# EvolEcolGroup/tidypopgen

Hardware: AMD Instinct MI355X
Metric: SNP-genotypes/s (N x M) for IBS+KING+GRM+Fst+PCA; max |delta| vs CPU ref (cpu_baseline.parity) (higher is better)
Workload: dtype fp4-e2m1 operands (exact integers, f32 accumulate) for the cross-products, the PCA Gram and the grouped counts, int8 (int32 accumulate) for the loadings, f64 for statistics

## Files before the change

### tidypopgen_amd/csrc/fst.hip

```cpp
#include <math.h>

#include <algorithm>

#include "common.h"
#include "devfrag.h"
#include "fst_terms.h"
#include "host/host_fsttiles.h"
typedef double v2d __attribute__((ext_vector_type(2)));

template <int METHOD, bool FAST, int PPT>
__global__ __launch_bounds__(256) void tpg_fst_kernel(FstSrc src, int64_t m, int G, int LB,
                                                      const int32_t* __restrict__ pairs0, int P, int by_locus,
                                                      int return_num_dem, double* __restrict__ part,
                                                      double* __restrict__ out_a, double* __restrict__ out_b) {
  extern __shared__ __attribute__((aligned(16))) double sh[];
  double* sh_n = sh;
  double* sh_p = sh + (size_t)LB * G;
  double* sh_h = sh + 2 * (size_t)LB * G;
  double* sh_e = sh + 3 * (size_t)LB * G;
  int pidx[PPT], g1[PPT], g2[PPT];
  double sum_num[PPT], sum_den[PPT];
#pragma unroll
  for (int k = 0; k < PPT; k++) {
    pidx[k] = (blockIdx.y * PPT + k) * 256 + threadIdx.x;
    g1[k] = 0; g2[k] = 0;
    if (pidx[k] < P) { g1[k] = pairs0[2 * pidx[k]]; g2[k] = pairs0[2 * pidx[k] + 1]; }
    sum_num[k] = 0.0; sum_den[k] = 0.0;
  }
  const int64_t nchunks = (m + LB - 1) / LB;
  for (int64_t ch = blockIdx.x; ch < nchunks; ch += gridDim.x) {
    const int64_t j0 = ch * LB;
    __syncthreads();
    for (int idx = threadIdx.x; idx < LB * G; idx += 256) {
      const int l = idx / G, g = idx % G;
      const int64_t j = j0 + l;
      double vn = FST_NAN, vp = FST_NAN, vh = FST_NAN;
      if (j < m) fst_stage(src, m, j, g, vn, vp, vh);
      sh_n[idx] = vn; sh_p[idx] = vp; sh_h[idx] = vh;
      if (METHOD == TPG_FST_HUDSON) sh_e[idx] = (vp * (1 - vp)) / (vn - 1);
      if (METHOD == TPG_FST_WC84 && FAST) {
        const double ni = 0.5 * vn;
        sh_n[idx] = ni; sh_h[idx] = vh * ni; sh_e[idx] = 1.0 / ni;
      }
    }
    __syncthreads();
    const int lmax = (int)((m - j0) < LB ? (m - j0) : LB);
#pragma unroll
    for (int k = 0; k < PPT; k++) {
      if (pidx[k] >= P) continue;
#pragma unroll 2
      for (int l = 0; l < lmax; l++) {
        const int o1 = l * G + g1[k], o2 = l * G + g2[k];
        double num, den;
        constexpr bool use_e = METHOD == TPG_FST_HUDSON || (METHOD == TPG_FST_WC84 && FAST);
        fst_terms<METHOD, FAST>(sh_n[o1], sh_p[o1], sh_h[o1], use_e ? sh_e[o1] : 0.0, sh_n[o2], sh_p[o2], sh_h[o2],
                                use_e ? sh_e[o2] : 0.0, num, den);
        if (!FAST && by_locus) {
          const int64_t o = (j0 + l) + (int64_t)pidx[k] * m;
          if (!return_num_dem) out_a[o] = num / den;
          else { out_a[o] = num; out_b[o] = den; }
        }
        if (num == num && den == den) { sum_num[k] += num; sum_den[k] += den; }
      }
    }
  }
#pragma unroll
  for (int k = 0; k < PPT; k++)
    if (pidx[k] < P) {
      part[((int64_t)blockIdx.x * P + pidx[k]) * 2] = sum_num[k];
      part[((int64_t)blockIdx.x * P + pidx[k]) * 2 + 1] = sum_den[k];
    }
}

__global__ __launch_bounds__(256) void tpg_fst_reduce_kernel(const double* __restrict__ part, int nblocks, int P,
                                                             double* __restrict__ fst_tot, double* __restrict__ sum_num,
                                                             double* __restrict__ sum_den) {
  __shared__ double shn[16][17], shd[16][17];
  const int px = threadIdx.x & 15, sl = threadIdx.x >> 4;
  const int pi = blockIdx.x * 16 + px;
  double sn = 0.0, sd = 0.0;
  if (pi < P)
    for (int b = sl; b < nblocks; b += 16) { sn += part[((int64_t)b * P + pi) * 2]; sd += part[((int64_t)b * P + pi) * 2 + 1]; }
  shn[sl][px] = sn; shd[sl][px] = sd;
  __syncthreads();
  if (sl == 0 && pi < P) {
    sn = 0.0; sd = 0.0;
    for (int t = 0; t < 16; t++) { sn += shn[t][px]; sd += shd[t][px]; }
    if (fst_tot) fst_tot[pi] = sn / sd;
    if (sum_num) { sum_num[pi] = sn; sum_den[pi] = sd; }
  }
}

#define FSTG_T 64
#define FSTG_LB 16
#define FSTG_RS_MFMA 80
__global__ __launch_bounds__(256) void tpg_fst_hudson_gemm_kernel(FstSrc src, int64_t m, int G, int ntile, int kmax,
                                                                  double* __restrict__ part) {
  extern __shared__ __attribute__((aligned(16))) double sh[];
  constexpr int RS = FSTG_RS_MFMA;
  double* ra = sh;
  double* rc = sh + FSTG_LB * RS;
  double* cb = sh + 2 * FSTG_LB * RS;
  const int tR = blockIdx.y / ntile, tC = blockIdx.y % ntile;
  const bool diag = tR == tC;
  double* cc = diag ? rc : sh + 3 * FSTG_LB * RS;
  double* inv = sh + 4 * FSTG_LB * RS;
  for (int A = threadIdx.x; A <= kmax; A += 256) { inv[2 * A] = 1.0 / (double)A; inv[2 * A + 1] = 1.0 / ((double)A - 1.0); }
  double AB[4][4], CB[4][4], CC[4][4];
#pragma unroll
  for (int r = 0; r < 4; r++)
#pragma unroll
    for (int c = 0; c < 4; c++) { AB[r][c] = 0.0; CB[r][c] = 0.0; CC[r][c] = 0.0; }
  const int lane = threadIdx.x & 63, wv = threadIdx.x >> 6, r16 = lane & 15, kq = lane >> 4;
  const int64_t nchunks = (m + FSTG_LB - 1) / FSTG_LB;
  constexpr int NSLOT = 2 * FSTG_LB * FSTG_T / 256;
  const int nslot = (diag ? 1 : 2) * FSTG_LB * FSTG_T / 256;
  int pn1[NSLOT], pn2[NSLOT], pnv[NSLOT];
  auto fetch = [&](int64_t ch) {
#pragma unroll
    for (int i = 0; i < NSLOT; i++) {
      pn1[i] = 0; pn2[i] = 0; pnv[i] = 0;
      if (i < nslot && ch < nchunks) {
        const int idx = threadIdx.x + 256 * i;
        const int side = idx / (FSTG_LB * FSTG_T), rem = idx % (FSTG_LB * FSTG_T);
        const int g = (side ? tC : tR) * FSTG_T + rem % FSTG_T;
        const int64_t j = ch * FSTG_LB + rem / FSTG_T;
        if (j < m && g < G) {
          const int64_t plane = src.Mpad * src.Cpad, o = j * src.Cpad + g;
          pn1[i] = src.cnt[o]; pn2[i] = src.cnt[plane + o]; pnv[i] = src.cnt[2 * plane + o];
        }
      }
    }
  };
  if (kmax > 0) fetch(blockIdx.x);
  for (int64_t ch = blockIdx.x; ch < nchunks; ch += gridDim.x) {
    const int64_t j0 = ch * FSTG_LB;
    __syncthreads();
    if (kmax > 0) {
#pragma unroll
      for (int i = 0; i < NSLOT; i++) {
        if (i >= nslot) break;
        const int idx = threadIdx.x + 256 * i;
        const int side = idx / (FSTG_LB * FSTG_T), rem = idx % (FSTG_LB * FSTG_T);
        double a = 0.0, b = 0.0, c = 0.0;
        const int A = min(2 * pnv[i], kmax);
        if (A > 0) {
          const double vp = (double)(pn1[i] + 2 * pn2[i]) * inv[2 * A];
          const double e = (vp * (1 - vp)) * inv[2 * A + 1];
          if (e == e) { a = vp * vp - e; b = 1.0; c = vp; }
        }
        const int srem = (rem / FSTG_T) * RS + rem % FSTG_T;
        if (side) { cb[srem] = b; cc[srem] = c; }
        else {
          ra[srem] = a; rc[srem] = c;
          if (diag) cb[srem] = b;
        }
      }
    } else {
      for (int idx = threadIdx.x; idx < (diag ? 1 : 2) * FSTG_LB * FSTG_T; idx += 256) {
        const int side = idx / (FSTG_LB * FSTG_T), rem = idx % (FSTG_LB * FSTG_T);
        const int l = rem / FSTG_T, gl = rem % FSTG_T;
        const int g = (side ? tC : tR) * FSTG_T + gl;
        const int64_t j = j0 + l;
        double a = 0.0, b = 0.0, c = 0.0;
        if (j < m && g < G) {
          double vn, vp, vh;
          fst_stage(src, m, j, g, vn, vp, vh);
          const double e = (vp * (1 - vp)) / (vn - 1);
          if (vp == vp && e == e) { a = vp * vp - e; b = 1.0; c = vp; }
        }
        const int srem = l * RS + gl;
        if (side) { cb[srem] = b; cc[srem] = c; }
        else {
          ra[srem] = a; rc[srem] = c;
          if (diag) cb[srem] = b;
        }
      }
    }
    __syncthreads();
    if (kmax > 0) fetch(ch + gridDim.x);
#pragma unroll
    for (int l = 0; l < FSTG_LB; l += 4) {
      const double av = ra[(l + kq) * RS + 16 * wv + r16], cv = rc[(l + kq) * RS + 16 * wv + r16];
#pragma unroll
      for (int ct = 0; ct < 4; ct++) {
        const double bv = cb[(l + kq) * RS + 16 * ct + r16], dv = cc[(l + kq) * RS + 16 * ct + r16];
        *(v4d*)AB[ct] = __builtin_amdgcn_mfma_f64_16x16x4f64(av, bv, *(v4d*)AB[ct], 0, 0, 0);
        *(v4d*)CB[ct] = __builtin_amdgcn_mfma_f64_16x16x4f64(cv, bv, *(v4d*)CB[ct], 0, 0, 0);
        *(v4d*)CC[ct] = __builtin_amdgcn_mfma_f64_16x16x4f64(cv, dv, *(v4d*)CC[ct], 0, 0, 0);
      }
    }
  }
  double* o = part + (((int64_t)blockIdx.x * gridDim.y + blockIdx.y) * 3) * FSTG_T * FSTG_T;
#pragma unroll
  for (int ct = 0; ct < 4; ct++)
#pragma unroll
    for (int reg = 0; reg < 4; reg++) {
      const int q = (16 * wv + kq + 4 * reg) * FSTG_T + 16 * ct + r16;
      o[q] = AB[ct][reg];
      o[FSTG_T * FSTG_T + q] = CB[ct][reg];
      o[2 * FSTG_T * FSTG_T + q] = CC[ct][reg];
    }
}

#define FSTG_SL 16
__global__ __launch_bounds__(256) void tpg_fst_hudson_gemm_reduce_kernel(const double* __restrict__ part, int nbx, int64_t cells,
                                                                         double* __restrict__ full) {
  const int64_t q = blockIdx.x * (int64_t)blockDim.x + threadIdx.x;
  if (q >= cells) return;
  double s = 0.0;
  for (int b = blockIdx.y; b < nbx; b += FSTG_SL) s += part[(int64_t)b * cells + q];
  full[(int64_t)blockIdx.y * cells + q] = s;
}

__global__ void tpg_fst_hudson_gemm_final_kernel(const double* __restrict__ full, int64_t cells, int ntile,
                                                 const int32_t* __restrict__ pairs0, int P, double* __restrict__ fst_tot,
                                                 double* __restrict__ sum_num, double* __restrict__ sum_den) {
  const int pi = blockIdx.x * blockDim.x + threadIdx.x;
  if (pi >= P) return;
  const int g1 = pairs0[2 * pi], g2 = pairs0[2 * pi + 1];
  auto at = [&](int prod, int r, int c) {
    const int t = (r / FSTG_T) * ntile + c / FSTG_T;
    const int64_t q = (((int64_t)t * 3 + prod) * FSTG_T + r % FSTG_T) * FSTG_T + c % FSTG_T;
    double v = 0.0;
    for (int sl = 0; sl < FSTG_SL; sl++) v += full[(int64_t)sl * cells + q];
    return v;
  };
  const double cc2 = 2 * at(2, g1, g2);
  const double sn = at(0, g1, g2) + at(0, g2, g1) - cc2, sd = at(1, g1, g2) + at(1, g2, g1) - cc2;
  if (fst_tot) fst_tot[pi] = sn / sd;
  if (sum_num) { sum_num[pi] = sn; sum_den[pi] = sd; }
}

#define FSTW_TAB 4
template <int PPT, int GS>
__global__ __launch_bounds__(256) void tpg_fst_wc84_tab_kernel(FstSrc src, int64_t m, int G, int LB, int kmax,
                                                               const int32_t* __restrict__ pairs0, int P,
                                                               double* __restrict__ part) {
  extern __shared__ __attribute__((aligned(16))) double sh[];
  const int gs = GS ? GS : G;
  const uint32_t sb_b = (uint32_t)LB * gs * 16u, tab_b = (uint32_t)LB * gs * 32u, tab2_b = tab_b + (uint32_t)(kmax + 1) * 16u;
  char* shb = (char*)sh;
  for (int A = threadIdx.x; A <= kmax; A += 256) {
    const double nt = 0.5 * (double)A, nb1 = 0.5 * nt - 1.0;
    const double r = 1.0 / nt, sv = 1.0 / nb1;
    double* t = (double*)(shb + tab_b) + (size_t)A * 2;
    t[0] = r;
    t[1] = (0.5 * (nt - 1.0)) * r;
    double* t2 = (double*)(shb + tab2_b) + (size_t)A * 2;
    t2[0] = (0.5 * nt) * sv;
    t2[1] = (0.25 * (nt * nt)) * sv;
  }
  int pidx[PPT];
  uint32_t o1[PPT], o2[PPT];
  double sum_num[PPT], sum_den[PPT];
#pragma unroll
  for (int k = 0; k < PPT; k++) {
    pidx[k] = (blockIdx.y * PPT + k) * 256 + threadIdx.x;
    o1[k] = 0; o2[k] = 0;
    if (pidx[k] < P) { o1[k] = (uint32_t)pairs0[2 * pidx[k]]; o2[k] = (uint32_t)pairs0[2 * pidx[k] + 1]; }
    sum_num[k] = 0.0; sum_den[k] = 0.0;
  }
  const int64_t nchunks = (m + LB - 1) / LB;
  constexpr int FSTW_SLOTS = 8;
  int pn1[FSTW_SLOTS], pn2[FSTW_SLOTS], pnv[FSTW_SLOTS];
  auto fetch = [&](int64_t ch) {
    const int64_t plane = src.Mpad * src.Cpad;
#pragma unroll
    for (int i = 0; i < FSTW_SLOTS; i++) {
      pn1[i] = 0; pn2[i] = 0; pnv[i] = 0;
      const int idx = threadIdx.x + 256 * i;
      if (idx < LB * G && ch < nchunks) {
        const int64_t j = ch * LB + idx / G;
        if (j < m) {
          const int64_t o = j * src.Cpad + idx % G;
          pn1[i] = src.cnt[o]; pn2[i] = src.cnt[plane + o]; pnv[i] = src.cnt[2 * plane + o];
        }
      }
    }
  };
  fetch(blockIdx.x);
  for (int64_t ch = blockIdx.x; ch < nchunks; ch += gridDim.x) {
    const int64_t j0 = ch * LB;
    __syncthreads();
#pragma unroll
    for (int i = 0; i < FSTW_SLOTS; i++) {
      const int idx = threadIdx.x + 256 * i;
      if (idx < LB * G) {
        const double vn = (double)(2 * pnv[i]);
        const double vp = (double)(pn1[i] + 2 * pn2[i]) / vn, vh = (double)(2 * pn1[i]) / vn;
        const double ni = 0.5 * vn;
        const uint32_t q = (uint32_t)((idx / G) * gs + idx % G);
        *(v2d*)(shb + q * 16u) = v2d{ni, vp};
        *(v2d*)(shb + sb_b + q * 16u) = v2d{vh * ni, 1.0 / ni};
      }
    }
    __syncthreads();
    fetch(ch + gridDim.x);
    const int lmax = (int)((m - j0) < LB ? (m - j0) : LB);
#pragma unroll
    for (int k = 0; k < PPT; k++) {
      if (pidx[k] >= P) continue;
      const uint32_t a1 = o1[k] * 16u, a2 = o2[k] * 16u;
      double sn = sum_num[k], sd = sum_den[k];
#pragma unroll 4
      for (int l = 0; l < lmax; l++) {
#pragma clang fp contract(fast)
        const uint32_t lo = (uint32_t)l * (uint32_t)gs;
        const v2d s1a = *(const v2d*)(shb + a1 + lo * 16u), s2a = *(const v2d*)(shb + a2 + lo * 16u);
        const v2d s1b = *(const v2d*)(shb + sb_b + a1 + lo * 16u), s2b = *(const v2d*)(shb + sb_b + a2 + lo * 16u);
        const v4d s1 = v4d{s1a[0], s1a[1], s1b[0], s1b[1]}, s2 = v4d{s2a[0], s2a[1], s2b[0], s2b[1]};
        const int A = min(__double2int_rz(2.0 * (s1[0] + s2[0])), kmax);
        const v2d ta = *(const v2d*)(shb + tab_b + (uint32_t)A * 16u), tb = *(const v2d*)(shb + tab2_b + (uint32_t)A * 16u);
        const v4d t = v4d{ta[0], ta[1], tb[0], tb[1]};
        const double p_bar = fma(s2[1], s2[0], s1[1] * s1[0]) * t[0], h_bar = (s1[2] + s2[2]) * t[0];
        const double d = s1[1] - s2[1], d2 = d * d;
        const double half_s2 = (d2 * (s1[0] * s2[0])) * (t[0] * t[0]);
        const double core = fma(-p_bar, p_bar, p_bar) - half_s2;
        const double X = t[3] * (s1[3] * s2[3]);
        const double a = fma(-X, fma(-0.25, h_bar, core), 0.5 * d2);
        const double b = t[2] * fma(-t[1], h_bar, core);
        const double den = fma(0.5, h_bar, a + b);
        if (den == den) { sn += a; sd += den; }
      }
      sum_num[k] = sn; sum_den[k] = sd;
    }
  }
#pragma unroll
  for (int k = 0; k < PPT; k++)
    if (pidx[k] < P) {
      part[((int64_t)blockIdx.x * P + pidx[k]) * 2] = sum_num[k];
      part[((int64_t)blockIdx.x * P + pidx[k]) * 2 + 1] = sum_den[k];
    }
}

#define FSTT_KMAX 511
#define FSTT_LB 16
#define FSTT_TAB2 (512 * 16)
#define FSTT_SA (2 * 512 * 16)
#define FSTT_SB (FSTT_SA + FSTT_LB * 64 * 16)
#define FSTT_LDS (FSTT_SB + FSTT_LB * 64 * 16)
__global__ __launch_bounds__(256, 3) void tpg_fst_wc84_tile_kernel(FstSrc src, int64_t m, int G, int kmax,
                                                                   const int32_t* __restrict__ tasks, int ntask, int P,
                                                                   double* __restrict__ part) {
  __shared__ __attribute__((aligned(16))) char shb[FSTT_LDS];
  constexpr int NPT = FSTW_TR * FSTW_TC, LB = FSTT_LB, GS = 64;
  for (int A = threadIdx.x; A <= kmax; A += 256) {
    const double nt = 0.5 * (double)A, nb1 = 0.5 * nt - 1.0;
    const double r = 1.0 / nt, sv = 1.0 / nb1;
    double* t = (double*)shb + (size_t)A * 2;
    t[0] = r * 0.03125;
    t[1] = (0.5 * (nt - 1.0)) * r;
    double* t2 = (double*)(shb + FSTT_TAB2) + (size_t)A * 2;
    t2[0] = (0.5 * nt) * sv;
    t2[1] = (0.25 * (nt * nt)) * sv;
  }
  const int task = blockIdx.y * 256 + threadIdx.x;
  const bool active = task < ntask;
  int pidx[NPT];
  uint32_t ro[FSTW_TR], co[FSTW_TC];
  double sum_num[NPT], sum_den[NPT];
  {
    const int r0 = active ? tasks[task * FSTW_TASK_INTS] : 0, c0 = active ? tasks[task * FSTW_TASK_INTS + 1] : 0;
#pragma unroll
    for (int i = 0; i < FSTW_TR; i++) ro[i] = (uint32_t)min(r0 + i, G - 1) * 16u;
#pragma unroll
    for (int j = 0; j < FSTW_TC; j++) co[j] = (uint32_t)min(c0 + j, G - 1) * 16u;
#pragma unroll
    for (int k = 0; k < NPT; k++) {
      pidx[k] = active ? tasks[task * FSTW_TASK_INTS + 2 + k] : -1;
      sum_num[k] = 0.0; sum_den[k] = 0.0;
    }
  }
  const int64_t nchunks = (m + LB - 1) / LB;
  constexpr int SLOTS = LB * GS / 256;
  int pn1[SLOTS], pn2[SLOTS], pnv[SLOTS];
  auto fetch = [&](int64_t ch) {
    const int64_t plane = src.Mpad * src.Cpad;
#pragma unroll
    for (int i = 0; i < SLOTS; i++) {
      pn1[i] = 0; pn2[i] = 0; pnv[i] = 0;
      if ((int)(threadIdx.x & 63u) < G && ch < nchunks) {
        const int64_t j = ch * LB + (threadIdx.x >> 6) + 4 * i;
        if (j < m) {
          const int64_t o = j * src.Cpad + (threadIdx.x & 63u);
          pn1[i] = src.cnt[o]; pn2[i] = src.cnt[plane + o]; pnv[i] = src.cnt[2 * plane + o];
        }
      }
    }
  };
  typedef __attribute__((address_space(3))) const char lchar;
  typedef __attribute__((address_space(3))) const v2d lv2d;
  auto locus = [&](lchar* const* pr, lchar* const* pc, auto off) {
#pragma clang fp contract(fast)
    constexpr int OFF = decltype(off)::value;
    v4d R[FSTW_TR], Cc[FSTW_TC];
#pragma unroll
    for (int i = 0; i < FSTW_TR; i++) {
      const v2d a = *(lv2d*)(pr[i] + OFF), b = *(lv2d*)(pr[i] + OFF + (FSTT_SB - FSTT_SA));
      R[i] = v4d{a[0], a[1], b[0], b[1]};
    }
#pragma unroll
    for (int j = 0; j < FSTW_TC; j++) {
      const v2d a = *(lv2d*)(pc[j] + OFF), b = *(lv2d*)(pc[j] + OFF + (FSTT_SB - FSTT_SA));
      Cc[j] = v4d{a[0], a[1], b[0], b[1]};
    }
    double av[NPT], dv[NPT];
    bool ok = true;
#pragma unroll
    for (int i = 0; i < FSTW_TR; i++)
#pragma unroll
      for (int j = 0; j < FSTW_TC; j++) {
        const int k = i * FSTW_TC + j;
        const v4d s1 = R[i], s2 = Cc[j];
        const int A16 = __double2int_rz(s1[0] + s2[0]);
        const v2d ta = *(const v2d*)(shb + A16), tb = *(const v2d*)(shb + A16 + FSTT_TAB2);
        const v4d t = v4d{ta[0], ta[1], tb[0], tb[1]};
        const double p_bar = fma(s2[1], s2[0], s1[1] * s1[0]) * t[0], h_bar = (s1[2] + s2[2]) * t[0];
        const double d = s1[1] - s2[1], d2 = d * d;
        const double half_s2 = (d2 * (s1[0] * s2[0])) * (t[0] * t[0]);
        const double core = fma(-p_bar, p_bar, p_bar) - half_s2;
        const double X = t[3] * (s1[3] * s2[3]);
        const double a = fma(-X, fma(-0.25, h_bar, core), 0.5 * d2);
        const double b = t[2] * fma(-t[1], h_bar, core);
        const double den = fma(0.5, h_bar, a + b);
        av[k] = a; dv[k] = den;
        ok = ok && den == den;
      }
    if (__all(ok)) {
#pragma unroll
      for (int k = 0; k < NPT; k++) { sum_num[k] += av[k]; sum_den[k] += dv[k]; }
    } else {
#pragma unroll
      for (int k = 0; k < NPT; k++)
        if (dv[k] == dv[k]) { sum_num[k] += av[k]; sum_den[k] += dv[k]; }
    }
  };
  fetch(blockIdx.x);
  for (int64_t ch = blockIdx.x; ch < nchunks; ch += gridDim.x) {
    const int64_t j0 = ch * LB;
    __syncthreads();
#pragma unroll
    for (int i = 0; i < SLOTS; i++) {
      if ((int)(threadIdx.x & 63u) < G) {
        const int nv = min(pnv[i], kmax >> 2);
        const double rn = 32.0 * *(const double*)(shb + (uint32_t)nv * 32u);
        const double ni = (double)nv;
        const double vp = (double)(pn1[i] + 2 * pn2[i]) * (0.5 * rn);
        const uint32_t q = threadIdx.x + 256u * (uint32_t)i;
        *(v2d*)(shb + FSTT_SA + q * 16u) = v2d{32.0 * ni, vp};
        *(v2d*)(shb + FSTT_SB + q * 16u) = v2d{32.0 * (double)pn1[i], rn};
      }
    }
    __syncthreads();
    fetch(ch + gridDim.x);
    const int lmax = (int)((m - j0) < LB ? (m - j0) : LB);
    if (!active) continue;
    lchar *pr[FSTW_TR], *pc[FSTW_TC];
#pragma unroll
    for (int i = 0; i < FSTW_TR; i++) pr[i] = (lchar*)(shb + FSTT_SA + ro[i]);
#pragma unroll
    for (int j = 0; j < FSTW_TC; j++) pc[j] = (lchar*)(shb + FSTT_SA + co[j]);
    int l = 0;
    for (; l + 2 <= lmax; l += 2) {
      locus(pr, pc, std::integral_constant<int, 0>{});
      locus(pr, pc, std::integral_constant<int, GS * 16>{});
#pragma unroll
      for (int i = 0; i < FSTW_TR; i++) pr[i] += 2 * GS * 16;
#pragma unroll
      for (int j = 0; j < FSTW_TC; j++) pc[j] += 2 * GS * 16;
    }
    if (l < lmax) locus(pr, pc, std::integral_constant<int, 0>{});
  }
#pragma unroll
  for (int k = 0; k < NPT; k++)
    if (pidx[k] >= 0) {
      part[((int64_t)blockIdx.x * P + pidx[k]) * 2] = sum_num[k];
      part[((int64_t)blockIdx.x * P + pidx[k]) * 2 + 1] = sum_den[k];
    }
}

__global__ void tpg_freq_ref_check_kernel(const double* __restrict__ p, const double* __restrict__ q, int64_t total,
                                          int* __restrict__ flag) {
  for (int64_t idx = blockIdx.x * (int64_t)blockDim.x + threadIdx.x; idx < total; idx += (int64_t)gridDim.x * blockDim.x) {
    const double want = 1 - p[idx], got = q[idx];
    if (!(want == got || (want != want && got != got))) flag[0] = 1;
  }
}

static int run_fst(tpg_ctx* ctx, int method, FstSrc src, int64_t m, int G, const int32_t* pairs1, int P, int by_locus,
                   int return_num_dem, double* fst_tot, double* out_a, double* out_b, double* sum_num = nullptr,
                   double* sum_den = nullptr, int kmax = 0 ) {
  TPG_REQUIRE(method == TPG_FST_HUDSON || method == TPG_FST_NEI87 || method == TPG_FST_WC84, TPG_EINVAL,
              "unknown Fst method %d", method);
  TPG_REQUIRE(P > 0 && pairs1, TPG_EINVAL, "no population pairs");
  if (return_num_dem) by_locus = 1;
  TPG_REQUIRE(!by_locus || out_a, TPG_EINVAL, "by_locus output requested but out_a is NULL");
  TPG_REQUIRE(!return_num_dem || out_b, TPG_EINVAL, "return_num_dem requested but out_b is NULL");
  TPG_REQUIRE(return_num_dem || fst_tot || sum_num, TPG_EINVAL, "fst_tot is NULL");
  TPG_REQUIRE((sum_num == nullptr) == (sum_den == nullptr), TPG_EINVAL, "sum_num and sum_den go together");
  std::vector<int32_t> p0((size_t)2 * P);
  for (int k = 0; k < 2 * P; k++) {
    TPG_REQUIRE(pairs1[k] >= 1 && pairs1[k] <= G, TPG_EINVAL, "pairwise_combn[%d] = %d out of [1,%d]", k, pairs1[k], G);
    p0[(size_t)k] = pairs1[k] - 1;
  }
  InBuf pb;
  TPG_TRY(pb.init(ctx, p0.data(), sizeof(int32_t) * 2 * (size_t)P));
  int LB = 32;
  while (LB > 1 && (size_t)LB * G * 4 * sizeof(double) > 96 * 1024) LB /= 2;
  TPG_REQUIRE((size_t)LB * G * 4 * sizeof(double) <= 150 * 1024, TPG_EUNSUPPORTED, "too many populations (%d)", G);
  const size_t shmem = (size_t)LB * G * 4 * sizeof(double);
  const bool fast = !by_locus;
  if (fast && method == TPG_FST_HUDSON) {
    const int ntile = (int)ceil_div(G, FSTG_T);
    const int64_t cells = (int64_t)ntile * ntile * 3 * FSTG_T * FSTG_T;
    const int64_t nch = ceil_div(m, FSTG_LB);
    int nbx = (int)std::min<int64_t>(nch, std::max(1, 4 * ctx->num_cu / (ntile * ntile)));
    OutBuf ot, osn, osd;
    if (fst_tot) TPG_TRY(ot.init(fst_tot, sizeof(double) * (size_t)P));
    if (sum_num) { TPG_TRY(osn.init(sum_num, sizeof(double) * (size_t)P)); TPG_TRY(osd.init(sum_den, sizeof(double) * (size_t)P)); }
    DevBuf gp;
    TPG_TRY(gp.alloc_n<double>((size_t)cells * (size_t)(nbx + FSTG_SL)));
    double* const d_gp = gp.as<double>();
    double* d_full = d_gp + (size_t)cells * (size_t)nbx;
    const int kq = (src.cnt && !src.has_hap && kmax > 0 && kmax <= 4096) ? kmax : 0;
    const size_t shg = sizeof(double) * (4 * FSTG_LB * FSTG_RS_MFMA + 2 * ((size_t)kq + 1));
    (void)hipFuncSetAttribute((const void*)tpg_fst_hudson_gemm_kernel, hipFuncAttributeMaxDynamicSharedMemorySize, (int)shg);
    TPG_LAUNCH(ctx, "fst_hudson", tpg_fst_hudson_gemm_kernel, dim3((unsigned)nbx, (unsigned)(ntile * ntile)), dim3(256), shg,
               src, m, G, ntile, kq, d_gp);
    TPG_LAUNCH(ctx, "fst_reduce", tpg_fst_hudson_gemm_reduce_kernel, dim3((unsigned)ceil_div(cells, 256), FSTG_SL), dim3(256), 0,
               (const double*)d_gp, nbx, cells, d_full);
    TPG_LAUNCH(ctx, "fst_reduce", tpg_fst_hudson_gemm_final_kernel, dim3((unsigned)ceil_div(P, 256)), dim3(256), 0, (const double*)d_full,
               cells, ntile, pb.dev<int32_t>(), P, ot.dev<double>(), osn.dev<double>(), osd.dev<double>());
    TPG_CHECK_LAUNCH();
    gp.free();
    if (fst_tot) TPG_TRY(ot.commit(ctx));
    if (sum_num) { TPG_TRY(osn.commit(ctx)); TPG_TRY(osd.commit(ctx)); }
    return TPG_OK;
  }
  const int64_t nchunks = ceil_div(m, LB);
  const int ppt = P > 256 ? 8 : 1;
  const int ypass = (int)ceil_div(P, 256 * ppt);
  int nblocks = (int)(nchunks < 4 * ctx->num_cu ? nchunks : 4 * ctx->num_cu);
  if (nblocks < 1) nblocks = 1;
  DevBuf part;
  TPG_TRY(part.alloc_n<double>(2 * (size_t)nblocks * (size_t)P));
  double* const d_part = part.as<double>();
  OutBuf ot, oa, ob, osn, osd;
  if (sum_num) { TPG_TRY(osn.init(sum_num, sizeof(double) * (size_t)P)); TPG_TRY(osd.init(sum_den, sizeof(double) * (size_t)P)); }
  const size_t mp = sizeof(double) * (size_t)m * (size_t)P;
  if (fst_tot) TPG_TRY(ot.init(fst_tot, sizeof(double) * (size_t)P));
  if (by_locus) TPG_TRY(oa.init(out_a, mp));
  if (return_num_dem) TPG_TRY(ob.init(out_b, mp));
  const int gs_tab = G <= 64 ? 64 : G, lb_tab = G <= 64 ? 16 : LB;
  const size_t sh_tab = (size_t)lb_tab * gs_tab * 32 + (size_t)(kmax + 1) * FSTW_TAB * 8;
  const bool wc84_tab = fast && method == TPG_FST_WC84 && src.cnt && !src.has_hap && kmax > 0 && sh_tab <= 150 * 1024 &&
                        (int64_t)lb_tab * G <= 8 * 256;
  if (wc84_tab) {
    const int64_t nch = ceil_div(m, lb_tab);
    const int nbt = (int)std::max<int64_t>(1, std::min<int64_t>(nch, (int64_t)nblocks));
    dim3 grid((unsigned)nbt, (unsigned)ypass);
    static const bool no_tiles = tpg_env_int("TPG_FST_TILES", 1) == 0;
    InBuf tb;
    int ntask = 0;
    const bool tiles = ppt == 8 && !no_tiles && G <= 64 && kmax <= FSTT_KMAX && lb_tab == FSTT_LB;
    if (tiles) {
      std::vector<int32_t> tasks;
      fst_wc84_tiles(p0, P, tasks);
      ntask = (int)(tasks.size() / FSTW_TASK_INTS);
      TPG_TRY(tb.init(ctx, tasks.data(), sizeof(int32_t) * tasks.size()));
    }
    if (ntask > 0) {
      const int nbt2 = (int)std::max<int64_t>(1, std::min<int64_t>(nch, (int64_t)nblocks));
      dim3 tgrid((unsigned)nbt2, (unsigned)ceil_div(ntask, 256));
      TPG_LAUNCH(ctx, "fst_wc84", tpg_fst_wc84_tile_kernel, tgrid, dim3(256), 0, src, m, G, kmax, tb.dev<int32_t>(), ntask, P,
                 d_part);
    } else {
#define FSTW_LAUNCH(PP, GSV)                                                                                                    \
  do {                                                                                                                          \
    (void)hipFuncSetAttribute((const void*)tpg_fst_wc84_tab_kernel<PP, GSV>, hipFuncAttributeMaxDynamicSharedMemorySize, (int)sh_tab); \
    TPG_LAUNCH(ctx, "fst_wc84", (tpg_fst_wc84_tab_kernel<PP, GSV>), grid, dim3(256), sh_tab, src, m, G, lb_tab, kmax, pb.dev<int32_t>(), P, \
               d_part);                                                                                                         \
  } while (0)
    if (ppt == 8 && G <= 64) FSTW_LAUNCH(8, 64);
    else if (ppt == 8) FSTW_LAUNCH(8, 0);
    else if (G <= 64) FSTW_LAUNCH(1, 64);
    else FSTW_LAUNCH(1, 0);
#undef FSTW_LAUNCH
    }
    TPG_LAUNCH(ctx, "fst_reduce", tpg_fst_reduce_kernel, dim3((unsigned)ceil_div(P, 16)), dim3(256), 0, d_part, nbt, P,
               ot.dev<double>(), osn.dev<double>(), osd.dev<double>());
  } else {
    dim3 grid((unsigned)nblocks, (unsigned)ypass);
#define FST_LAUNCH1(M, F, PP, NAME)                                                                              \
  do {                                                                                                           \
    (void)hipFuncSetAttribute((const void*)tpg_fst_kernel<M, F, PP>, hipFuncAttributeMaxDynamicSharedMemorySize,  \
                              (int)shmem);                                                                       \
    TPG_LAUNCH(ctx, NAME, (tpg_fst_kernel<M, F, PP>), grid, dim3(256), shmem, src, m, G, LB, pb.dev<int32_t>(), P, \
               by_locus, return_num_dem, d_part, oa.dev<double>(), ob.dev<double>());                            \
  } while (0)
#define FST_LAUNCH(M, F, NAME) do { if (ppt == 8) FST_LAUNCH1(M, F, 8, NAME); else FST_LAUNCH1(M, F, 1, NAME); } while (0)
    if (method == TPG_FST_HUDSON && fast) FST_LAUNCH(TPG_FST_HUDSON, true, "fst_hudson");
    else if (method == TPG_FST_HUDSON) FST_LAUNCH(TPG_FST_HUDSON, false, "fst_hudson");
    else if (method == TPG_FST_WC84 && fast) FST_LAUNCH(TPG_FST_WC84, true, "fst_wc84");
    else if (method == TPG_FST_WC84) FST_LAUNCH(TPG_FST_WC84, false, "fst_wc84");
    else FST_LAUNCH(TPG_FST_NEI87, false, "fst_nei87");
#undef FST_LAUNCH1
#undef FST_LAUNCH
    if (fst_tot || sum_num)
      TPG_LAUNCH(ctx, "fst_reduce", tpg_fst_reduce_kernel, dim3((unsigned)ceil_div(P, 16)), dim3(256), 0, d_part,
                 nblocks, P, ot.dev<double>(), osn.dev<double>(), osd.dev<double>());
  }
  TPG_CHECK_LAUNCH();
  part.free();
  if (fst_tot) TPG_TRY(ot.commit(ctx));
  if (sum_num) { TPG_TRY(osn.commit(ctx)); TPG_TRY(osd.commit(ctx)); }
  if (by_locus) TPG_TRY(oa.commit(ctx));
  if (return_num_dem) TPG_TRY(ob.commit(ctx));
  return TPG_OK;
}

extern "C" int tpg_pairwise_fst_loop(tpg_ctx* ctx, int method, const int32_t* pairs1, int P, int64_t m, int G,
                                     const double* n, const double* freq_alt, const double* freq_ref,
                                     const double* het_obs, int by_locus, int return_num_dem, double* fst_tot,
                                     double* out_a, double* out_b) {
  TpgEnter _enter(ctx);
  TPG_REQUIRE(ctx && n && freq_alt, TPG_EINVAL, "null argument");
  TPG_REQUIRE(m > 0 && G > 0, TPG_EINVAL, "empty input");
  TPG_REQUIRE(method == TPG_FST_HUDSON || het_obs, TPG_EINVAL, "het_obs is required for WC84 / Nei87");
  const size_t bytes = sizeof(double) * (size_t)m * (size_t)G;
  InBuf bn, bp, bh;
  TPG_TRY(bn.init(ctx, n, bytes));
  TPG_TRY(bp.init(ctx, freq_alt, bytes));
  if (het_obs) TPG_TRY(bh.init(ctx, het_obs, bytes));
  if (freq_ref && method != TPG_FST_WC84) {
    InBuf bq;
    TPG_TRY(bq.init(ctx, freq_ref, bytes));
    DevBuf d_bad;
    TPG_TRY(d_bad.alloc_n<int>(1));
    int bad = 0;
    TPG_HIP(hipMemsetAsync(d_bad.p, 0, sizeof(int), ctx->stream));
    TPG_LAUNCH(ctx, "freq_ref_check", tpg_freq_ref_check_kernel, dim3(1024), dim3(256), 0, bp.dev<double>(), bq.dev<double>(),
               (int64_t)m * G, d_bad.as<int>());
    TPG_HIP(tpg_fetch_small(ctx, &bad, d_bad.p, sizeof(int)));
    TPG_REQUIRE(!bad, TPG_EINVAL, "freq_ref is not 1 - freq_alt: the device path recomputes it and would not match the reference");
  }
  FstSrc src{nullptr, 0, 0, 0, bn.dev<double>(), bp.dev<double>(), nullptr, het_obs ? bh.dev<double>() : nullptr};
  return run_fst(ctx, method, src, m, G, pairs1, P, by_locus, return_num_dem, fst_tot, out_a, out_b);
}

static int fused_fst(tpg_ctx* ctx, const tpg_view* v, const int32_t* groupIds0, int ngroups, const double* ploidy,
                     int method, const int32_t* pairs1, int P, int by_locus, int return_num_dem, double* fst_tot,
                     double* out_a, double* out_b, double* sum_num, double* sum_den) {
  TPG_REQUIRE(ctx && v && groupIds0, TPG_EINVAL, "null argument");
  ClassPlan cp;
  TPG_TRY(make_class_plan(v->n, groupIds0, ngroups, ploidy, &cp));
  TPG_REQUIRE(!cp.has_hap || method == TPG_FST_HUDSON, TPG_EINVAL,
              "only method = Hudson is valid when the data include pseudohaploids");
  GroupedCounts gc;
  TPG_TRY(tpg_grouped_counts(ctx, v, cp.cls.data(), cp.nclass, &gc));
  FstSrc src{gc.cnt, gc.Mpad, gc.Cpad, cp.has_hap, nullptr, nullptr, nullptr, nullptr};
  const int64_t kmax = 4 * (int64_t)*std::max_element(cp.group_size.begin(), cp.group_size.end());
  return run_fst(ctx, method, src, v->m, ngroups, pairs1, P, by_locus, return_num_dem, fst_tot, out_a, out_b, sum_num,
                 sum_den, kmax < (1 << 20) ? (int)kmax : 0);
}

extern "C" int tpg_pairwise_pop_fst(tpg_ctx* ctx, const tpg_view* v, const int32_t* groupIds0, int ngroups,
                                    const double* ploidy, int method, const int32_t* pairs1, int P, int by_locus,
                                    int return_num_dem, double* fst_tot, double* out_a, double* out_b) {
  TpgEnter _enter(ctx);
  return fused_fst(ctx, v, groupIds0, ngroups, ploidy, method, pairs1, P, by_locus, return_num_dem, fst_tot, out_a,
                   out_b, nullptr, nullptr);
}

extern "C" int tpg_pairwise_pop_fst_sums(tpg_ctx* ctx, const tpg_view* v, const int32_t* groupIds0, int ngroups,
                                         const double* ploidy, int method, const int32_t* pairs1, int P,
                                         double* sum_num, double* sum_den) {
  TpgEnter _enter(ctx);
  TPG_REQUIRE(sum_num && sum_den, TPG_EINVAL, "null output");
  return fused_fst(ctx, v, groupIds0, ngroups, ploidy, method, pairs1, P, 0, 0, nullptr, nullptr, nullptr, sum_num,
                   sum_den);
}

__global__ void tpg_pbs_kernel(const double* __restrict__ fst, int64_t m, const int32_t* __restrict__ trip, int ntrip,
                               double* __restrict__ out) {
  const int64_t total = m * ntrip;
  for (int64_t idx = blockIdx.x * (int64_t)blockDim.x + threadIdx.x; idx < total;
       idx += (int64_t)gridDim.x * blockDim.x) {
    const int64_t j = idx % m;
    const int t = (int)(idx / m);
    const double f12 = fst[j + (int64_t)trip[3 * t] * m], f13 = fst[j + (int64_t)trip[3 * t + 1] * m],
                 f23 = fst[j + (int64_t)trip[3 * t + 2] * m];
    const double t12 = -log(1 - f12), t13 = -log(1 - f13), t23 = -log(1 - f23);
    const double p1 = (t12 + t13 - t23) / 2, p2 = (t12 + t23 - t13) / 2, p3 = (t13 + t23 - t12) / 2;
    double* o = out + (int64_t)t * 6 * m + j;
    o[0] = p1; o[m] = p2; o[2 * m] = p3;
    o[3 * m] = p1 / (1 + p1 + p2 + p3);
    o[4 * m] = p2 / (1 + p1 + p2 + p3);
    o[5 * m] = p3 / (1 + p1 + p2 + p3);
  }
}

extern "C" int tpg_pbs_from_fst(tpg_ctx* ctx, const double* fst, int64_t m, int P, const int32_t* trip_cols0, int ntrip,
                                double* out) {
  TpgEnter _enter(ctx);
  TPG_REQUIRE(ctx && fst && trip_cols0 && out, TPG_EINVAL, "null argument");
  TPG_REQUIRE(m > 0 && P > 0 && ntrip > 0, TPG_EINVAL, "bad sizes");
  for (int k = 0; k < 3 * ntrip; k++)
    TPG_REQUIRE(trip_cols0[k] >= 0 && trip_cols0[k] < P, TPG_EINVAL, "triplet column %d out of [0,%d)", trip_cols0[k], P);
  InBuf ifst, itr;
  TPG_TRY(ifst.init(ctx, fst, sizeof(double) * (size_t)m * (size_t)P));
  TPG_TRY(itr.init(ctx, trip_cols0, sizeof(int32_t) * 3 * (size_t)ntrip));
  OutBuf o;
  TPG_TRY(o.init(out, sizeof(double) * (size_t)m * 6 * (size_t)ntrip));
  TPG_LAUNCH(ctx, "pbs", tpg_pbs_kernel, dim3(2048), dim3(256), 0, ifst.dev<double>(), m, itr.dev<int32_t>(), ntrip,
             o.dev<double>());
  TPG_CHECK_LAUNCH();
  TPG_HIP(hipStreamSynchronize(ctx->stream));
  return o.commit(ctx);
}
```

Baseline: 140.4 billion.

## Restructure Hudson GEMM with masked complement and add reduced WC84 pair formula

The Hudson Fst GEMM now assumes loci are valid by default. It accumulates unmasked row sums (SA, SC) through a single MFMA against a per-locus validity vector, and runs the AB/CB cross-product MFMAs only for chunks flagged as containing missing entries, using a complement correction. This replaces two of the three per-tile MFMA products on clean data. The WC84 tile kernel gains a templated reduced path, used when every group has at least three members, with a simpler algebraic per-pair formula, a smaller table and int sample counts. It falls back to the full formula when a NaN appears. The changes add flag bookkeeping in LDS and numerical-parity risk from the rearranged arithmetic.

```diff
diff --git a/tidypopgen_amd/csrc/fst.hip b/tidypopgen_amd/csrc/fst.hip
--- a/tidypopgen_amd/csrc/fst.hip
+++ b/tidypopgen_amd/csrc/fst.hip
@@ -94,6 +94,7 @@
 #define FSTG_T 64
 #define FSTG_LB 16
 #define FSTG_RS_MFMA 80
+#define FSTG_TS (3 * FSTG_T * FSTG_T + 2 * FSTG_T)
 __global__ __launch_bounds__(256) void tpg_fst_hudson_gemm_kernel(FstSrc src, int64_t m, int G, int ntile, int kmax,
                                                                   double* __restrict__ part) {
   extern __shared__ __attribute__((aligned(16))) double sh[];
@@ -106,11 +107,16 @@
   double* cc = diag ? rc : sh + 3 * FSTG_LB * RS;
   double* inv = sh + 4 * FSTG_LB * RS;
   for (int A = threadIdx.x; A <= kmax; A += 256) { inv[2 * A] = 1.0 / (double)A; inv[2 * A + 1] = 1.0 / ((double)A - 1.0); }
-  double AB[4][4], CB[4][4], CC[4][4];
-#pragma unroll
-  for (int r = 0; r < 4; r++)
-#pragma unroll
-    for (int c = 0; c < 4; c++) { AB[r][c] = 0.0; CB[r][c] = 0.0; CC[r][c] = 0.0; }
+  int* flag = (int*)(inv + 2 * ((size_t)kmax + 1));
+  constexpr int FS = FSTG_LB + 1;
+  if (threadIdx.x < 2 * FS) flag[threadIdx.x] = 0;
+  double AD[4][4], CD[4][4], CC[4][4], SA[4], SC[4];
+#pragma unroll
+  for (int r = 0; r < 4; r++) {
+    SA[r] = 0.0; SC[r] = 0.0;
+#pragma unroll
+    for (int c = 0; c < 4; c++) { AD[r][c] = 0.0; CD[r][c] = 0.0; CC[r][c] = 0.0; }
+  }
   const int lane = threadIdx.x & 63, wv = threadIdx.x >> 6, r16 = lane & 15, kq = lane >> 4;
   const int64_t nchunks = (m + FSTG_LB - 1) / FSTG_LB;
   constexpr int NSLOT = 2 * FSTG_LB * FSTG_T / 256;
@@ -119,7 +125,7 @@
   auto fetch = [&](int64_t ch) {
 #pragma unroll
     for (int i = 0; i < NSLOT; i++) {
-      pn1[i] = 0; pn2[i] = 0; pnv[i] = 0;
+      pn1[i] = 0; pn2[i] = 0; pnv[i] = -1;
       if (i < nslot && ch < nchunks) {
         const int idx = threadIdx.x + 256 * i;
         const int side = idx / (FSTG_LB * FSTG_T), rem = idx % (FSTG_LB * FSTG_T);
@@ -133,28 +139,31 @@
     }
   };
   if (kmax > 0) fetch(blockIdx.x);
-  for (int64_t ch = blockIdx.x; ch < nchunks; ch += gridDim.x) {
+  int par = 0;
+  for (int64_t ch = blockIdx.x; ch < nchunks; ch += gridDim.x, par ^= 1) {
     const int64_t j0 = ch * FSTG_LB;
     __syncthreads();
+    if (threadIdx.x < FS) flag[(par ^ 1) * FS + threadIdx.x] = 0;
     if (kmax > 0) {
 #pragma unroll
       for (int i = 0; i < NSLOT; i++) {
         if (i >= nslot) break;
         const int idx = threadIdx.x + 256 * i;
         const int side = idx / (FSTG_LB * FSTG_T), rem = idx % (FSTG_LB * FSTG_T);
-        double a = 0.0, b = 0.0, c = 0.0;
+        double a = 0.0, u = pnv[i] >= 0 ? 1.0 : 0.0, c = 0.0;
         const int A = min(2 * pnv[i], kmax);
         if (A > 0) {
           const double vp = (double)(pn1[i] + 2 * pn2[i]) * inv[2 * A];
           const double e = (vp * (1 - vp)) * inv[2 * A + 1];
-          if (e == e) { a = vp * vp - e; b = 1.0; c = vp; }
+          if (e == e) { a = vp * vp - e; u = 0.0; c = vp; }
         }
         const int srem = (rem / FSTG_T) * RS + rem % FSTG_T;
-        if (side) { cb[srem] = b; cc[srem] = c; }
+        if (side) { cb[srem] = u; cc[srem] = c; }
         else {
           ra[srem] = a; rc[srem] = c;
-          if (diag) cb[srem] = b;
-        }
+          if (diag) cb[srem] = u;
+        }
+        if ((side || diag) && u != 0.0) { flag[par * FS + rem / FSTG_T] = 1; flag[par * FS + FSTG_LB] = 1; }
       }
     } else {
       for (int idx = threadIdx.x; idx < (diag ? 1 : 2) * FSTG_LB * FSTG_T; idx += 256) {
@@ -162,44 +171,67 @@
         const int l = rem / FSTG_T, gl = rem % FSTG_T;
         const int g = (side ? tC : tR) * FSTG_T + gl;
         const int64_t j = j0 + l;
-        double a = 0.0, b = 0.0, c = 0.0;
+        double a = 0.0, u = 0.0, c = 0.0;
         if (j < m && g < G) {
           double vn, vp, vh;
           fst_stage(src, m, j, g, vn, vp, vh);
           const double e = (vp * (1 - vp)) / (vn - 1);
-          if (vp == vp && e == e) { a = vp * vp - e; b = 1.0; c = vp; }
+          if (vp == vp && e == e) { a = vp * vp - e; c = vp; }
+          else u = 1.0;
         }
         const int srem = l * RS + gl;
-        if (side) { cb[srem] = b; cc[srem] = c; }
+        if (side) { cb[srem] = u; cc[srem] = c; }
         else {
           ra[srem] = a; rc[srem] = c;
-          if (diag) cb[srem] = b;
-        }
+          if (diag) cb[srem] = u;
+        }
+        if ((side || diag) && u != 0.0) { flag[par * FS + l] = 1; flag[par * FS + FSTG_LB] = 1; }
       }
     }
     __syncthreads();
     if (kmax > 0) fetch(ch + gridDim.x);
+    const int* dirty = flag + par * FS;
 #pragma unroll
     for (int l = 0; l < FSTG_LB; l += 4) {
       const double av = ra[(l + kq) * RS + 16 * wv + r16], cv = rc[(l + kq) * RS + 16 * wv + r16];
+      const double kv = dirty[l + kq] ? 0.0 : 1.0;
+      *(v4d*)SA = __builtin_amdgcn_mfma_f64_16x16x4f64(av, kv, *(v4d*)SA, 0, 0, 0);
+      *(v4d*)SC = __builtin_amdgcn_mfma_f64_16x16x4f64(cv, kv, *(v4d*)SC, 0, 0, 0);
 #pragma unroll
       for (int ct = 0; ct < 4; ct++) {
-        const double bv = cb[(l + kq) * RS + 16 * ct + r16], dv = cc[(l + kq) * RS + 16 * ct + r16];
-        *(v4d*)AB[ct] = __builtin_amdgcn_mfma_f64_16x16x4f64(av, bv, *(v4d*)AB[ct], 0, 0, 0);
-        *(v4d*)CB[ct] = __builtin_amdgcn_mfma_f64_16x16x4f64(cv, bv, *(v4d*)CB[ct], 0, 0, 0);
+        const double dv = cc[(l + kq) * RS + 16 * ct + r16];
         *(v4d*)CC[ct] = __builtin_amdgcn_mfma_f64_16x16x4f64(cv, dv, *(v4d*)CC[ct], 0, 0, 0);
       }
     }
-  }
-  double* o = part + (((int64_t)blockIdx.x * gridDim.y + blockIdx.y) * 3) * FSTG_T * FSTG_T;
+    if (dirty[FSTG_LB]) {
+#pragma unroll
+      for (int l = 0; l < FSTG_LB; l += 4) {
+        const double av = ra[(l + kq) * RS + 16 * wv + r16], cv = rc[(l + kq) * RS + 16 * wv + r16];
+        const bool d = dirty[l + kq] != 0;
+#pragma unroll
+        for (int ct = 0; ct < 4; ct++) {
+          const double bv = d ? 1.0 - cb[(l + kq) * RS + 16 * ct + r16] : 0.0;
+          *(v4d*)AD[ct] = __builtin_amdgcn_mfma_f64_16x16x4f64(av, bv, *(v4d*)AD[ct], 0, 0, 0);
+          *(v4d*)CD[ct] = __builtin_amdgcn_mfma_f64_16x16x4f64(cv, bv, *(v4d*)CD[ct], 0, 0, 0);
+        }
+      }
+    }
+  }
+  double* o = part + ((int64_t)blockIdx.x * gridDim.y + blockIdx.y) * FSTG_TS;
 #pragma unroll
   for (int ct = 0; ct < 4; ct++)
 #pragma unroll
     for (int reg = 0; reg < 4; reg++) {
       const int q = (16 * wv + kq + 4 * reg) * FSTG_T + 16 * ct + r16;
-      o[q] = AB[ct][reg];
-      o[FSTG_T * FSTG_T + q] = CB[ct][reg];
+      o[q] = AD[ct][reg];
+      o[FSTG_T * FSTG_T + q] = CD[ct][reg];
       o[2 * FSTG_T * FSTG_T + q] = CC[ct][reg];
+    }
+  if (r16 == 0)
+#pragma unroll
+    for (int reg = 0; reg < 4; reg++) {
+      o[3 * FSTG_T * FSTG_T + 16 * wv + kq + 4 * reg] = SA[reg];
+      o[3 * FSTG_T * FSTG_T + FSTG_T + 16 * wv + kq + 4 * reg] = SC[reg];
     }
 }
 
@@ -219,15 +251,21 @@
   const int pi = blockIdx.x * blockDim.x + threadIdx.x;
   if (pi >= P) return;
   const int g1 = pairs0[2 * pi], g2 = pairs0[2 * pi + 1];
-  auto at = [&](int prod, int r, int c) {
-    const int t = (r / FSTG_T) * ntile + c / FSTG_T;
-    const int64_t q = (((int64_t)t * 3 + prod) * FSTG_T + r % FSTG_T) * FSTG_T + c % FSTG_T;
+  auto cell = [&](int64_t q) {
     double v = 0.0;
     for (int sl = 0; sl < FSTG_SL; sl++) v += full[(int64_t)sl * cells + q];
     return v;
   };
+  auto at = [&](int prod, int r, int c) {
+    const int t = (r / FSTG_T) * ntile + c / FSTG_T;
+    return cell(((int64_t)t * FSTG_TS + (prod * FSTG_T + r % FSTG_T) * FSTG_T) + c % FSTG_T);
+  };
+  auto masked = [&](int k, int r, int c) {
+    const int t = (r / FSTG_T) * ntile + c / FSTG_T;
+    return cell((int64_t)t * FSTG_TS + 3 * FSTG_T * FSTG_T + k * FSTG_T + r % FSTG_T) + at(k, r, c);
+  };
   const double cc2 = 2 * at(2, g1, g2);
-  const double sn = at(0, g1, g2) + at(0, g2, g1) - cc2, sd = at(1, g1, g2) + at(1, g2, g1) - cc2;
+  const double sn = masked(0, g1, g2) + masked(0, g2, g1) - cc2, sd = masked(1, g1, g2) + masked(1, g2, g1) - cc2;
   if (fst_tot) fst_tot[pi] = sn / sd;
   if (sum_num) { sum_num[pi] = sn; sum_den[pi] = sd; }
 }
@@ -336,24 +374,53 @@
 
 #define FSTT_KMAX 511
 #define FSTT_LB 16
-#define FSTT_TAB2 (512 * 16)
-#define FSTT_SA (2 * 512 * 16)
-#define FSTT_SB (FSTT_SA + FSTT_LB * 64 * 16)
-#define FSTT_LDS (FSTT_SB + FSTT_LB * 64 * 16)
+#define FSTT_MIN_GROUP 3
+__device__ __forceinline__ void fstt_full_table(int A, double& t0, double& t1, double& t2, double& t3) {
+  const double nt = 0.5 * (double)A, nb1 = 0.5 * nt - 1.0;
+  const double r = 1.0 / nt, sv = 1.0 / nb1;
+  t0 = r * 0.03125;
+  t1 = (0.5 * (nt - 1.0)) * r;
+  t2 = (0.5 * nt) * sv;
+  t3 = (0.25 * (nt * nt)) * sv;
+}
+__device__ __forceinline__ void fstt_full_pair(const v4d s1, const v4d s2, const v4d t, double& a_out, double& den_out) {
+#pragma clang fp contract(fast)
+  const double p_bar = fma(s2[1], s2[0], s1[1] * s1[0]) * t[0], h_bar = (s1[2] + s2[2]) * t[0];
+  const double d = s1[1] - s2[1], d2 = d * d;
+  const double half_s2 = (d2 * (s1[0] * s2[0])) * (t[0] * t[0]);
+  const double core = fma(-p_bar, p_bar, p_bar) - half_s2;
+  const double X = t[3] * (s1[3] * s2[3]);
+  const double a = fma(-X, fma(-0.25, h_bar, core), 0.5 * d2);
+  const double b = t[2] * fma(-t[1], h_bar, core);
+  a_out = a;
+  den_out = fma(0.5, h_bar, a + b);
+}
+template <bool RED>
 __global__ __launch_bounds__(256, 3) void tpg_fst_wc84_tile_kernel(FstSrc src, int64_t m, int G, int kmax,
                                                                    const int32_t* __restrict__ tasks, int ntask, int P,
                                                                    double* __restrict__ part) {
-  __shared__ __attribute__((aligned(16))) char shb[FSTT_LDS];
   constexpr int NPT = FSTW_TR * FSTW_TC, LB = FSTT_LB, GS = 64;
+  constexpr int TAB2 = 512 * 16;
+  constexpr int SA = RED ? 512 * 16 : 2 * 512 * 16;
+  constexpr int SB = SA + LB * GS * 16;
+  constexpr int SN = SB + LB * GS * 16;
+  constexpr int LDS = RED ? SN + LB * GS * 4 : SN;
+  static_assert(LDS <= 53 * 1024, "three workgroups per CU");
+  __shared__ __attribute__((aligned(16))) char shb[LDS];
   for (int A = threadIdx.x; A <= kmax; A += 256) {
-    const double nt = 0.5 * (double)A, nb1 = 0.5 * nt - 1.0;
-    const double r = 1.0 / nt, sv = 1.0 / nb1;
-    double* t = (double*)shb + (size_t)A * 2;
-    t[0] = r * 0.03125;
-    t[1] = (0.5 * (nt - 1.0)) * r;
-    double* t2 = (double*)(shb + FSTT_TAB2) + (size_t)A * 2;
-    t2[0] = (0.5 * nt) * sv;
-    t2[1] = (0.25 * (nt * nt)) * sv;
+    if (RED) {
+      const double nt = 0.5 * (double)A;
+      double* t = (double*)shb + (size_t)A * 2;
+      t[0] = A > 4 ? 1.0 / (nt - 2.0) : FST_NAN;
+      t[1] = 1.0 / nt;
+    } else {
+      double t0, t1, t2, t3;
+      fstt_full_table(A, t0, t1, t2, t3);
+      double* t = (double*)shb + (size_t)A * 2;
+      t[0] = t0; t[1] = t1;
+      double* u = (double*)(shb + TAB2) + (size_t)A * 2;
+      u[0] = t2; u[1] = t3;
+    }
   }
   const int task = blockIdx.y * 256 + threadIdx.x;
   const bool active = task < ntask;
@@ -391,19 +458,23 @@
   };
   typedef __attribute__((address_space(3))) const char lchar;
   typedef __attribute__((address_space(3))) const v2d lv2d;
-  auto locus = [&](lchar* const* pr, lchar* const* pc, auto off) {
+  typedef __attribute__((address_space(3))) const int lint;
+  auto locus = [&](lchar* const* pr, lchar* const* pc, lchar* const* qr, lchar* const* qc, auto off) {
 #pragma clang fp contract(fast)
     constexpr int OFF = decltype(off)::value;
     v4d R[FSTW_TR], Cc[FSTW_TC];
+    int Rn[FSTW_TR], Cn[FSTW_TC];
 #pragma unroll
     for (int i = 0; i < FSTW_TR; i++) {
-      const v2d a = *(lv2d*)(pr[i] + OFF), b = *(lv2d*)(pr[i] + OFF + (FSTT_SB - FSTT_SA));
+      const v2d a = *(lv2d*)(pr[i] + OFF), b = *(lv2d*)(pr[i] + OFF + (SB - SA));
       R[i] = v4d{a[0], a[1], b[0], b[1]};
+      Rn[i] = RED ? *(lint*)(qr[i] + OFF / 4) : 0;
     }
 #pragma unroll
     for (int j = 0; j < FSTW_TC; j++) {
-      const v2d a = *(lv2d*)(pc[j] + OFF), b = *(lv2d*)(pc[j] + OFF + (FSTT_SB - FSTT_SA));
+      const v2d a = *(lv2d*)(pc[j] + OFF), b = *(lv2d*)(pc[j] + OFF + (SB - SA));
       Cc[j] = v4d{a[0], a[1], b[0], b[1]};
+      Cn[j] = RED ? *(lint*)(qc[j] + OFF / 4) : 0;
     }
     double av[NPT], dv[NPT];
     bool ok = true;
@@ -413,23 +484,40 @@
       for (int j = 0; j < FSTW_TC; j++) {
         const int k = i * FSTW_TC + j;
         const v4d s1 = R[i], s2 = Cc[j];
-        const int A16 = __double2int_rz(s1[0] + s2[0]);
-        const v2d ta = *(const v2d*)(shb + A16), tb = *(const v2d*)(shb + A16 + FSTT_TAB2);
-        const v4d t = v4d{ta[0], ta[1], tb[0], tb[1]};
-        const double p_bar = fma(s2[1], s2[0], s1[1] * s1[0]) * t[0], h_bar = (s1[2] + s2[2]) * t[0];
-        const double d = s1[1] - s2[1], d2 = d * d;
-        const double half_s2 = (d2 * (s1[0] * s2[0])) * (t[0] * t[0]);
-        const double core = fma(-p_bar, p_bar, p_bar) - half_s2;
-        const double X = t[3] * (s1[3] * s2[3]);
-        const double a = fma(-X, fma(-0.25, h_bar, core), 0.5 * d2);
-        const double b = t[2] * fma(-t[1], h_bar, core);
-        const double den = fma(0.5, h_bar, a + b);
-        av[k] = a; dv[k] = den;
-        ok = ok && den == den;
+        if (RED) {
+          const v2d t = *(const v2d*)(shb + (Rn[i] + Cn[j]));
+          const double d = s1[0] - s2[0], d2 = d * d;
+          const double cs = s1[1] + s2[1], hs = s1[2] + s2[2], en = s1[3] + s2[3];
+          const double w = t[0] * en;
+          av[k] = fma(-w, fma(-0.5, hs, cs), d2);
+          dv[k] = fma(t[0], fma(-t[1], hs, cs), av[k]);
+        } else {
+          const int A16 = __double2int_rz(s1[0] + s2[0]);
+          const v2d ta = *(const v2d*)(shb + A16), tb = *(const v2d*)(shb + A16 + TAB2);
+          fstt_full_pair(s1, s2, v4d{ta[0], ta[1], tb[0], tb[1]}, av[k], dv[k]);
+        }
+        ok = ok && dv[k] == dv[k];
       }
     if (__all(ok)) {
 #pragma unroll
       for (int k = 0; k < NPT; k++) { sum_num[k] += av[k]; sum_den[k] += dv[k]; }
+    } else if (RED) {
+#pragma unroll
+      for (int i = 0; i < FSTW_TR; i++)
+#pragma unroll
+        for (int j = 0; j < FSTW_TC; j++) {
+          const int k = i * FSTW_TC + j;
+          const v2d ra = *(lv2d*)(pr[i] + OFF), rb = *(lv2d*)(pr[i] + OFF + (SB - SA));
+          const v2d ca = *(lv2d*)(pc[j] + OFF), cb = *(lv2d*)(pc[j] + OFF + (SB - SA));
+          const int rn = *(lint*)(qr[i] + OFF / 4), cn = *(lint*)(qc[j] + OFF / 4);
+          const v4d s1 = v4d{(double)rn, ra[0], 32.0 * rb[0], 2.0 * rb[1]};
+          const v4d s2 = v4d{(double)cn, ca[0], 32.0 * cb[0], 2.0 * cb[1]};
+          double t0, t1, t2, t3, a, den;
+          fstt_full_table((rn + cn) >> 4, t0, t1, t2, t3);
+          fstt_full_pair(s1, s2, v4d{t0, t1, t2, t3}, a, den);
+          if (den == den) { sum_num[k] += 2.0 * a; sum_den[k] += 2.0 * den; }
+          __builtin_amdgcn_sched_barrier(0);
+        }
     } else {
 #pragma unroll
       for (int k = 0; k < NPT; k++)
@@ -444,39 +532,46 @@
     for (int i = 0; i < SLOTS; i++) {
       if ((int)(threadIdx.x & 63u) < G) {
         const int nv = min(pnv[i], kmax >> 2);
-        const double rn = 32.0 * *(const double*)(shb + (uint32_t)nv * 32u);
+        const double rn = RED ? *(const double*)(shb + (uint32_t)nv * 32u + 8u) : 32.0 * *(const double*)(shb + (uint32_t)nv * 32u);
         const double ni = (double)nv;
         const double vp = (double)(pn1[i] + 2 * pn2[i]) * (0.5 * rn);
         const uint32_t q = threadIdx.x + 256u * (uint32_t)i;
-        *(v2d*)(shb + FSTT_SA + q * 16u) = v2d{32.0 * ni, vp};
-        *(v2d*)(shb + FSTT_SB + q * 16u) = v2d{32.0 * (double)pn1[i], rn};
+        if (RED) {
+          *(v2d*)(shb + SA + q * 16u) = v2d{vp, ((2.0 * ni) * vp) * (1.0 - vp)};
+          *(v2d*)(shb + SB + q * 16u) = v2d{(double)pn1[i], 0.5 * rn};
+          *(int*)(shb + SN + q * 4u) = 32 * nv;
+        } else {
+          *(v2d*)(shb + SA + q * 16u) = v2d{32.0 * ni, vp};
+          *(v2d*)(shb + SB + q * 16u) = v2d{32.0 * (double)pn1[i], rn};
+        }
       }
     }
     __syncthreads();
     fetch(ch + gridDim.x);
     const int lmax = (int)((m - j0) < LB ? (m - j0) : LB);
     if (!active) continue;
-    lchar *pr[FSTW_TR], *pc[FSTW_TC];
-#pragma unroll
-    for (int i = 0; i < FSTW_TR; i++) pr[i] = (lchar*)(shb + FSTT_SA + ro[i]);
-#pragma unroll
-    for (int j = 0; j < FSTW_TC; j++) pc[j] = (lchar*)(shb + FSTT_SA + co[j]);
+    lchar *pr[FSTW_TR], *pc[FSTW_TC], *qr[FSTW_TR], *qc[FSTW_TC];
+#pragma unroll
+    for (int i = 0; i < FSTW_TR; i++) { pr[i] = (lchar*)(shb + SA + ro[i]); qr[i] = (lchar*)(shb + SN + (ro[i] >> 2)); }
+#pragma unroll
+    for (int j = 0; j < FSTW_TC; j++) { pc[j] = (lchar*)(shb + SA + co[j]); qc[j] = (lchar*)(shb + SN + (co[j] >> 2)); }
     int l = 0;
     for (; l + 2 <= lmax; l += 2) {
-      locus(pr, pc, std::integral_constant<int, 0>{});
-      locus(pr, pc, std::integral_constant<int, GS * 16>{});
-#pragma unroll
-      for (int i = 0; i < FSTW_TR; i++) pr[i] += 2 * GS * 16;
-#pragma unroll
-      for (int j = 0; j < FSTW_TC; j++) pc[j] += 2 * GS * 16;
-    }
-    if (l < lmax) locus(pr, pc, std::integral_constant<int, 0>{});
-  }
+      locus(pr, pc, qr, qc, std::integral_constant<int, 0>{});
+      locus(pr, pc, qr, qc, std::integral_constant<int, GS * 16>{});
+#pragma unroll
+      for (int i = 0; i < FSTW_TR; i++) { pr[i] += 2 * GS * 16; qr[i] += 2 * GS * 4; }
+#pragma unroll
+      for (int j = 0; j < FSTW_TC; j++) { pc[j] += 2 * GS * 16; qc[j] += 2 * GS * 4; }
+    }
+    if (l < lmax) locus(pr, pc, qr, qc, std::integral_constant<int, 0>{});
+  }
+  const double scale = RED ? 0.5 : 1.0;
 #pragma unroll
   for (int k = 0; k < NPT; k++)
     if (pidx[k] >= 0) {
-      part[((int64_t)blockIdx.x * P + pidx[k]) * 2] = sum_num[k];
-      part[((int64_t)blockIdx.x * P + pidx[k]) * 2 + 1] = sum_den[k];
+      part[((int64_t)blockIdx.x * P + pidx[k]) * 2] = scale * sum_num[k];
+      part[((int64_t)blockIdx.x * P + pidx[k]) * 2 + 1] = scale * sum_den[k];
     }
 }
 
@@ -490,7 +585,8 @@
 
 static int run_fst(tpg_ctx* ctx, int method, FstSrc src, int64_t m, int G, const int32_t* pairs1, int P, int by_locus,
                    int return_num_dem, double* fst_tot, double* out_a, double* out_b, double* sum_num = nullptr,
-                   double* sum_den = nullptr, int kmax = 0 ) {
+                   double* sum_den = nullptr, int kmax = 0 ,
+                   int gmin = 0 ) {
   TPG_REQUIRE(method == TPG_FST_HUDSON || method == TPG_FST_NEI87 || method == TPG_FST_WC84, TPG_EINVAL,
               "unknown Fst method %d", method);
   TPG_REQUIRE(P > 0 && pairs1, TPG_EINVAL, "no population pairs");
@@ -513,7 +609,7 @@
   const bool fast = !by_locus;
   if (fast && method == TPG_FST_HUDSON) {
     const int ntile = (int)ceil_div(G, FSTG_T);
-    const int64_t cells = (int64_t)ntile * ntile * 3 * FSTG_T * FSTG_T;
+    const int64_t cells = (int64_t)ntile * ntile * FSTG_TS;
     const int64_t nch = ceil_div(m, FSTG_LB);
     int nbx = (int)std::min<int64_t>(nch, std::max(1, 4 * ctx->num_cu / (ntile * ntile)));
     OutBuf ot, osn, osd;
@@ -524,7 +620,7 @@
     double* const d_gp = gp.as<double>();
     double* d_full = d_gp + (size_t)cells * (size_t)nbx;
     const int kq = (src.cnt && !src.has_hap && kmax > 0 && kmax <= 4096) ? kmax : 0;
-    const size_t shg = sizeof(double) * (4 * FSTG_LB * FSTG_RS_MFMA + 2 * ((size_t)kq + 1));
+    const size_t shg = sizeof(double) * (4 * FSTG_LB * FSTG_RS_MFMA + 2 * ((size_t)kq + 1) + FSTG_LB + 1);
     (void)hipFuncSetAttribute((const void*)tpg_fst_hudson_gemm_kernel, hipFuncAttributeMaxDynamicSharedMemorySize, (int)shg);
     TPG_LAUNCH(ctx, "fst_hudson", tpg_fst_hudson_gemm_kernel, dim3((unsigned)nbx, (unsigned)(ntile * ntile)), dim3(256), shg,
                src, m, G, ntile, kq, d_gp);
@@ -573,8 +669,12 @@
     if (ntask > 0) {
       const int nbt2 = (int)std::max<int64_t>(1, std::min<int64_t>(nch, (int64_t)nblocks));
       dim3 tgrid((unsigned)nbt2, (unsigned)ceil_div(ntask, 256));
-      TPG_LAUNCH(ctx, "fst_wc84", tpg_fst_wc84_tile_kernel, tgrid, dim3(256), 0, src, m, G, kmax, tb.dev<int32_t>(), ntask, P,
-                 d_part);
+      if (gmin >= FSTT_MIN_GROUP)
+        TPG_LAUNCH(ctx, "fst_wc84", tpg_fst_wc84_tile_kernel<true>, tgrid, dim3(256), 0, src, m, G, kmax, tb.dev<int32_t>(), ntask,
+                   P, d_part);
+      else
+        TPG_LAUNCH(ctx, "fst_wc84", tpg_fst_wc84_tile_kernel<false>, tgrid, dim3(256), 0, src, m, G, kmax, tb.dev<int32_t>(), ntask,
+                   P, d_part);
     } else {
 #define FSTW_LAUNCH(PP, GSV)                                                                                                    \
   do {                                                                                                                          \
@@ -661,8 +761,9 @@
   TPG_TRY(tpg_grouped_counts(ctx, v, cp.cls.data(), cp.nclass, &gc));
   FstSrc src{gc.cnt, gc.Mpad, gc.Cpad, cp.has_hap, nullptr, nullptr, nullptr, nullptr};
   const int64_t kmax = 4 * (int64_t)*std::max_element(cp.group_size.begin(), cp.group_size.end());
+  const int64_t gmin = *std::min_element(cp.group_size.begin(), cp.group_size.end());
   return run_fst(ctx, method, src, v->m, ngroups, pairs1, P, by_locus, return_num_dem, fst_tot, out_a, out_b, sum_num,
-                 sum_den, kmax < (1 << 20) ? (int)kmax : 0);
+                 sum_den, kmax < (1 << 20) ? (int)kmax : 0, (int)std::min<int64_t>(gmin, 1 << 20));
 }
 
 extern "C" int tpg_pairwise_pop_fst(tpg_ctx* ctx, const tpg_view* v, const int32_t* groupIds0, int ngroups,
```

Result: faster. 142.8 billion (median of 6 runs) (+1.7%).
